# CHAINNEVERLIU/Pytorch-RL-EnhancedStableBaselines

Hardware: AMD Instinct MI355X
Metric: env-steps/sec (SAC, two-series CSTR, 4096 vec-envs) at 1/2/4/8 GPUs (higher is better)
Workload: dtype f32; 1 GPU; SAC MlpPolicy class defaults on 4096 vectorised two-series CSTR envs per GPU (obs 4/act 2, euler, batch 256, ring 244x4096, 1 gradient step per vec-step; hipGraph replay, 8 iterations per graph); n_envs_per_gpu=4096, global_batch=256, parallelism=dp1, hip_graph=True, hip_graph_requested=True, graph_unroll=8, blas=rocblas, n_updates=2370

## Files before the change

### include/cstr_rl_hip.h

```cpp
#ifndef CSTR_RL_HIP_H
#define CSTR_RL_HIP_H

#include <stdint.h>

#ifdef __cplusplus
extern "C" {
#endif

#define CSTR_ABI_VERSION 5

#define CSTR_OK 0
#define CSTR_E_BADARG (-1)
#define CSTR_E_UNSUPPORTED (-2)

#define CSTR_INTEGRATOR_EULER 0
#define CSTR_INTEGRATOR_RK4 1

typedef void *cstr_stream_t;

typedef struct cstr_coef {
    float q_v1, q_v2, cf, tf, tcf, k0, neg_e, r_gas, hk, rho_cp, cool1, cool2, neg_ua1, neg_ua2, rho_c, c_pc, dt;
    float s_lo[4], s_hi[4], s_span[4];
    float a_lo[2], a_hi[2], a_span[2];
    float target_c2, conc_span;
// ... 198 lines not shown

int cstr_sac_alpha_f32(const float *log_alpha, const float *logp, float target_entropy, float *grad_out, float *ent_coef_out,
                       float *loss_out, float *loss_sum, float *ent_coef_sum, int64_t batch, cstr_stream_t stream);

int cstr_twin_q_loss_f32(const float *q1, const float *q2, const float *target, float scale, float *gq1, float *gq2,
                         float *loss_out, float *loss_sum, int64_t batch, cstr_stream_t stream);

typedef struct cstr_alpha_part {
    const float *log_alpha;
    const float *logp_pi;
    float target_entropy;
    float *grad_out;
    float *ent_coef_out;
    float *loss_out;
    float *loss_sum;
    float *ent_coef_sum;
} cstr_alpha_part_t;
int cstr_td_twin_q_loss_f32(const float *q1_t, const float *q2_t, const float *next_logp, const float *rew, const float *done,
                            const float *ent_coef, float gamma, const float *q1, const float *q2, float scale, float *target_out,
                            float *gq1, float *gq2, float *loss_out, float *loss_sum, const cstr_alpha_part_t *alpha,
                            int64_t batch, cstr_stream_t stream);

typedef struct cstr_head_root {
    int32_t mode, batch;
    float gamma, scale;
    const float *q1_t, *q2_t, *next_logp, *rew, *done;
    const float *ent_coef;
    const float *q1, *q2;
    float *target_out;
    const float *logp;
    float *g_logp;
    float *loss_out, *loss_sum;
    cstr_alpha_part_t alpha;
} cstr_head_root_t;
int cstr_hidden_head_bwd_root_f32(const cstr_head_root_t *root, const float *y, int act, const float *w2, float *dz, float *gb1,
                                  float *gw2, float *gb2, int64_t m, int64_t k, cstr_stream_t stream);

int cstr_sac_actor_loss_f32(const float *logp, const float *q1, const float *q2, const float *ent_coef, float *g_logp, float *gq1,
                            float *gq2, float *loss_out, float *loss_sum, int64_t batch, cstr_stream_t stream);

#define CSTR_MAX_ENS_CRITICS 16
int cstr_td_ens_q_loss_f32(const float *q_t, int64_t q_t_stride, const float *next_logp, const float *rew, const float *done,
                           const float *ent_coef, float gamma, const float *q, int64_t q_stride, float scale, float *target_out, float *gq,
                           float *loss_out, float *loss_sum, const cstr_alpha_part_t *alpha, int n_critics, int64_t batch,
                           cstr_stream_t stream);
int cstr_sac_actor_ens_loss_f32(const float *logp, const float *q, int64_t q_stride, const float *ent_coef, float *g_logp, float *gq,
                                float *loss_out, float *loss_sum, int n_critics, int64_t batch, cstr_stream_t stream);

#define CSTR_SDE_MAX_LATENT 4096
#define CSTR_SDE_MAX_MATS 65537
int cstr_sde_draw_f32(const float *log_std, int log_std_cols, int latent, int act_dim, int use_expln, int64_t n_mats, float *std_out,
                      float *z, int64_t z_keep, float *mats, uint64_t *rng_ctl, cstr_stream_t stream);
int cstr_sde_head_fwd_f32(const float *h, int64_t ldh, int64_t batch, int latent, int act_dim, const float *w_mu, const float *b_mu,
                          float clip_mean, const float *mats, int64_t mat_stride, const float *std_mat, float *action, int64_t action_stride,
                          float *logp, float *aux, cstr_stream_t stream);
int cstr_sde_head_bwd_f32(const float *g_action, int64_t g_action_stride, const float *g_logp, const float *action, int64_t action_stride,
                          const float *aux, const float *h, int64_t ldh, int64_t batch, int latent, int act_dim, const float *w_mu,
                          float clip_mean, const float *mats, int64_t mat_stride, const float *std_mat, int below_act, float *g_pre,
                          float *g_x, float *g_var, float *dh, cstr_stream_t stream);
int cstr_sde_param_grad_f32(const float *h, int64_t ldh, int64_t batch, int latent, int act_dim, const float *g_pre, const float *g_x,
                            const float *g_var, const float *z, const float *std_mat, const float *log_std, int log_std_cols, int use_expln,
                            float *dw_mu, float *db_mu, float *dlog_std, cstr_stream_t stream);

int cstr_neg_mean_loss_f32(const float *q, float *gq, float *loss_out, float *loss_sum, int64_t batch, cstr_stream_t stream);

typedef struct cstr_adam_opt {
    const int64_t *adam_ctl;
    const double *lr;
    double beta1, beta2, eps;
    float grad_scale;
    int32_t reserved;
} cstr_adam_opt_t;
typedef struct cstr_wgrad_adam_set {
    cstr_wgrad_set_t g;
    float *w, *w_m, *w_v;
    float *b, *b_m, *b_v;
    float *shadow;
    int32_t opt, reserved;
    float *w_target, *b_target;
    float tau, reserved2;
} cstr_wgrad_adam_set_t;
int cstr_linear_bwd_weight_adam_sets_f32(const cstr_wgrad_adam_set_t *sets, int n_sets, const cstr_adam_opt_t *opts, int n_opts,
                                         const cstr_adam_seg_t *flat, int n_flat, cstr_stream_t stream);

#define CSTR_CHAIN_MAX_NETS 16
#define CSTR_CHAIN_MAX_WIDTH 512

typedef struct cstr_chain_net {
    const float *w1, *b1, *w2, *b2, *w3, *b3;
    const float *x;
    float *h1, *h2;
    float *q_part;
    int32_t role, reserved;
} cstr_chain_net_t;
#define CSTR_CHAIN_ROLE_PLAIN 0
#define CSTR_CHAIN_ROLE_STORE_PI 1
#define CSTR_CHAIN_ROLE_NEXT 2
#define CSTR_CHAIN_ROLE_NEXT_STORE 3
#define CSTR_CHAIN_ROLE_PI 4
#define CSTR_CHAIN_ROWS_PAIR 0
#define CSTR_CHAIN_ROWS_NEXT 1
#define CSTR_CHAIN_ROWS_OBS 2
#define CSTR_CHAIN_HEAD_GAUSSIAN 0
#define CSTR_CHAIN_HEAD_DETERMINISTIC 1

typedef struct cstr_sac_actor {
    int32_t obs_dim, act_dim, h1, h2;
    const float *w1, *b1, *w2, *b2, *hw, *hb;
} cstr_sac_actor_t;

int cstr_sac_actor_chain_fwd_f32(const cstr_sac_actor_t *actor, const cstr_ring_t *ring, int64_t *ring_ctl, int advance_ring,
                                 const int32_t *sample_idx, int64_t batch, float *x_data, float *x_pi, float *x_next, float *out_done,
                                 float *out_rew, float *a_h1, float *a_h2, float *head_part, const uint64_t *head_rng_ctl,
                                 uint64_t head_rng_offset, float *eps_all, int rows_mode, int head_n, int tiles, cstr_stream_t stream);

typedef struct cstr_sac_head_fin {
    const float *head_part;
    const float *hb;
    const float *eps;
    int32_t n_parts, act_dim, obs_dim, kind;
    int32_t part_rows, next_offset;
    float sigma, clip;
    float *x_pi, *x_next;
    float *params, *logp_pi, *logp_next;
} cstr_sac_head_fin_t;

int cstr_q_chain_fwd_f32(const cstr_chain_net_t *nets, int n_nets, int w_in, int obs_dim, int h1, int h2, int64_t batch,
                         const cstr_sac_head_fin_t *fin, int tiles, cstr_stream_t stream);

typedef struct cstr_chain_root {
    int32_t mode, batch;
    float gamma, scale;
    const float *q_part[4];
    const float *b3[4];
    int32_t n_parts, reserved;
    const float *next_logp, *rew, *done;
    const float *ent_coef;
    const float *logp;
    float *target_out;
    float *q_out;
    float *gq_out;
    float *loss_out, *loss_sum;
    cstr_alpha_part_t alpha;
    uint64_t *rng_ctl;
    uint64_t rng_advance;
    int64_t *adam_advance[2];
    double adam_beta1[2], adam_beta2[2];
} cstr_chain_root_t;
int cstr_q_chain_bwd_f32(const cstr_chain_net_t *nets, int n_nets, const cstr_chain_root_t *root, int w_in, int obs_dim, int h1, int h2,
                         float *dz2, float *dz1, float *gact_part, int tiles, cstr_stream_t stream);

int cstr_chain_sum_parts_f32(const float *part, int n_parts, int64_t rows, int cols, float *out, int64_t out_stride, cstr_stream_t stream);

int cstr_sac_actor_chain_bwd_f32(const cstr_sac_actor_t *actor, const float *gact_part, int n_nets, int n_parts, const float *ent_coef,
                                 const float *x_pi, const float *params, const float *eps, const float *a_h1, const float *a_h2,
                                 float *g_params, float *dz2, float *dz1, int64_t batch, int kind, int tiles, cstr_stream_t stream);

#define CSTR_BCQ_MAX_LATENT 256
#define CSTR_BCQ_MAX_ACT 64
#define CSTR_BCQ_MAX_SAMPLES 4096
#define CSTR_BCQ_MAX_ROWS 16777216
int cstr_bcq_latent_fwd_f32(const float *params, int64_t ldp, const float *obs, int64_t ldo, const float *eps_in, uint64_t *rng_ctl,
                            float *xdec, int64_t ldx, float *std_out, float *eps_out, int64_t batch, int obs_dim, int latent,
                            cstr_stream_t stream);
int cstr_bcq_vae_loss_f32(const float *recon, int64_t ldr, const float *act, int64_t lda, const float *params, int64_t ldp,
                          const float *std, int64_t batch, int act_dim, int latent, float *g_recon, float *g_mean, float *g_std,
// ... 92 lines not shown
```

### pytorch-rl-enhancedstablebaselines_amd/core/_native.py

```python
import ctypes as C
import os
from typing import Optional

_PKG_ROOT = os.path.dirname(os.path.dirname(os.path.abspath(__file__)))
LIB_PATH = os.environ.get("CSTR_LIB_PATH", os.path.join(_PKG_ROOT, "libcstr_rl_hip.so"))

INTEGRATORS = {"euler": 0, "rk4": 1}
RING_CTL_WORDS, ADAM_CTL_WORDS, MT_STATE_WORDS, PCG_STATE_WORDS, MAX_SAMPLE_BATCH = 4, 4, 628, 4, 16384
MAX_NOISE_PERIOD = 8
VECNORM_STATE_WORDS = 20
RNG_CTL_WORDS, MAX_HEAD_ACT, MAX_LINEAR_SETS, MAX_ADAM_SEGS = 16, 4, 16, 4
MAX_ENS_CRITICS = 16
SDE_MAX_LATENT, SDE_MAX_MATS = 4096, 65537
BCQ_MAX_LATENT, BCQ_MAX_ACT, BCQ_MAX_SAMPLES, BCQ_MAX_ROWS = 256, 64, 4096, 1 << 24
ROLLOUT_CTL_WORDS, PPO_WS_WORDS, PPO_MAX_BLOCKS, PPO_MAX_ROWS = 4, 1024, 64, 1 << 30
DQN_MAX_LEVELS = 16

SYMBOLS = (
    "cstr_abi_version", "cstr_error_string", "cstr_default_coef", "cstr_vec_step_f32", "cstr_reset_draw_f32",
    "cstr_replay_add_f32", "cstr_collect_step_f32", "cstr_collect_step_rng_f32", "cstr_mt19937_seed", "cstr_mt19937_normal_f32", "cstr_mt19937_normal_f64", "cstr_replay_sample_mt19937_f32", "cstr_replay_sample_packed_mt19937_f32", "cstr_replay_gather_packed_f32", "cstr_rollout_step_f32", "cstr_linear_act_fwd_gather_f32",
    "cstr_adam_multi_f32", "cstr_gaussian_head_fwd_f32", "cstr_gaussian_head_gemm_fwd_f32", "cstr_gaussian_head_bwd_f32", "cstr_gaussian_head_bwd_input_f32", "cstr_linear_act_fwd_f32", "cstr_linear_act_fwd_sets_f32", "cstr_linear_bwd_input_f32", "cstr_linear_bwd_weight_f32", "cstr_linear_bwd_weight_sets_f32", "cstr_td_twin_q_loss_f32", "cstr_policy_rows_fwd_f32", "cstr_policy_swizzle_f32", "cstr_target_smooth_f32", "cstr_linear_smooth_fwd_f32", "cstr_hidden_head_fwd_f32", "cstr_hidden_head_bwd_f32", "cstr_hidden_head_bwd_root_f32", "cstr_vecnorm_init_f64", "cstr_vecnorm_step_f64", "cstr_vecnorm_apply_f32",
    "cstr_td_target_min_f32", "cstr_polyak_f32", "cstr_adam_f32", "cstr_bias_act_fwd_f32", "cstr_bias_act_bwd_f32", "cstr_bias_act_bwd_rows_f32",
    "cstr_squashed_gaussian_fwd_f32", "cstr_squashed_gaussian_bwd_f32", "cstr_sac_alpha_f32", "cstr_twin_q_loss_f32",
    "cstr_sac_actor_loss_f32", "cstr_neg_mean_loss_f32", "cstr_td_ens_q_loss_f32", "cstr_sac_actor_ens_loss_f32",
    "cstr_sac_actor_chain_fwd_f32", "cstr_q_chain_fwd_f32", "cstr_q_chain_bwd_f32", "cstr_sac_actor_chain_bwd_f32",
    "cstr_linear_bwd_weight_adam_sets_f32", "cstr_chain_sum_parts_f32",
    "cstr_sde_draw_f32", "cstr_sde_head_fwd_f32", "cstr_sde_head_bwd_f32", "cstr_sde_param_grad_f32",
    "cstr_bcq_latent_fwd_f32", "cstr_bcq_vae_loss_f32", "cstr_bcq_latent_bwd_f32", "cstr_bcq_expand_f32", "cstr_bcq_perturb_fwd_f32",
    "cstr_bcq_perturb_bwd_f32", "cstr_bcq_target_f32", "cstr_bcq_select_f32",
    "cstr_diag_gaussian_act_f32", "cstr_rollout_add_f32", "cstr_gae_f32", "cstr_ppo_gather_f32", "cstr_ppo_loss_f32", "cstr_grad_clip_f32",
    "cstr_a2c_loss_f32", "cstr_rmsprop_f32",
    "cstr_mt19937_rand_flag_f64", "cstr_dqn_act_f32", "cstr_dqn_loss_f32",
    "cstr_eval_episodes_f32",
)


class Coef(C.Structure):
    _fields_ = [(n, C.c_float) for n in (
        "q_v1", "q_v2", "cf", "tf", "tcf", "k0", "neg_e", "r_gas", "hk", "rho_cp", "cool1", "cool2", "neg_ua1",
        "neg_ua2", "rho_c", "c_pc", "dt")] + [
        ("s_lo", C.c_float * 4), ("s_hi", C.c_float * 4), ("s_span", C.c_float * 4),
        ("a_lo", C.c_float * 2), ("a_hi", C.c_float * 2), ("a_span", C.c_float * 2),
        ("target_c2", C.c_float), ("conc_span", C.c_float), ("max_steps", C.c_int32)]


class Ring(C.Structure):
    _fields_ = [(n, C.c_void_p) for n in ("obs", "next_obs", "act", "rew", "done", "timeout")] + [
        ("rows", C.c_int64), ("n_envs", C.c_int64), ("obs_dim", C.c_int32), ("act_dim", C.c_int32)]


class AdamSeg(C.Structure):
    _fields_ = [("param", C.c_void_p), ("grad", C.c_void_p), ("exp_avg", C.c_void_p), ("exp_avg_sq", C.c_void_p),
                ("adam_ctl", C.c_void_p), ("lr", C.c_void_p), ("beta1", C.c_double), ("beta2", C.c_double), ("eps", C.c_double),
                ("grad_scale", C.c_float), ("n", C.c_int64), ("polyak_source", C.c_void_p), ("tau", C.c_double),
                ("shadow", C.c_void_p), ("shadow_begin", C.c_int64), ("shadow_n", C.c_int64), ("shadow_k", C.c_int64), ("own_target", C.c_void_p)]


class LinearSet(C.Structure):
    _fields_ = [("x", C.c_void_p), ("ldx", C.c_int64), ("w", C.c_void_p), ("bias", C.c_void_p), ("y", C.c_void_p), ("ldy", C.c_int64)]


class WgradSet(C.Structure):
    _fields_ = [("dz", C.c_void_p), ("x", C.c_void_p), ("ldx", C.c_int64), ("dw", C.c_void_p), ("db", C.c_void_p),
                ("m", C.c_int64), ("n", C.c_int64), ("k", C.c_int64)]


class AlphaPart(C.Structure):
    _fields_ = [("log_alpha", C.c_void_p), ("logp_pi", C.c_void_p), ("target_entropy", C.c_float), ("grad_out", C.c_void_p),
                ("ent_coef_out", C.c_void_p), ("loss_out", C.c_void_p), ("loss_sum", C.c_void_p), ("ent_coef_sum", C.c_void_p)]


class HeadRoot(C.Structure):
    _fields_ = [("mode", C.c_int32), ("batch", C.c_int32), ("gamma", C.c_float), ("scale", C.c_float), ("q1_t", C.c_void_p),
                ("q2_t", C.c_void_p), ("next_logp", C.c_void_p), ("rew", C.c_void_p), ("done", C.c_void_p), ("ent_coef", C.c_void_p),
                ("q1", C.c_void_p), ("q2", C.c_void_p), ("target_out", C.c_void_p), ("logp", C.c_void_p), ("g_logp", C.c_void_p),
                ("loss_out", C.c_void_p), ("loss_sum", C.c_void_p), ("alpha", AlphaPart)]


class PolicyMlp(C.Structure):
    _fields_ = [("k0", C.c_int32), ("h1", C.c_int32), ("h2", C.c_int32), ("act_dim", C.c_int32), ("act", C.c_int32), ("head", C.c_int32),
                ("out_act", C.c_int32), ("reserved", C.c_int32), ("w1", C.c_void_p), ("b1", C.c_void_p), ("w2", C.c_void_p),
                ("b2", C.c_void_p), ("w3", C.c_void_p), ("b3", C.c_void_p), ("w2_swizzled", C.c_void_p)]


CHAIN_MAX_NETS, CHAIN_MAX_WIDTH = 16, 512
CHAIN_ROLE_PLAIN, CHAIN_ROLE_STORE_PI, CHAIN_ROLE_NEXT, CHAIN_ROLE_NEXT_STORE, CHAIN_ROLE_PI = 0, 1, 2, 3, 4
CHAIN_ROWS_PAIR, CHAIN_ROWS_NEXT, CHAIN_ROWS_OBS = 0, 1, 2
CHAIN_HEAD_GAUSSIAN, CHAIN_HEAD_DETERMINISTIC = 0, 1


class ChainNet(C.Structure):
    _fields_ = [(n, C.c_void_p) for n in ("w1", "b1", "w2", "b2", "w3", "b3", "x", "h1", "h2", "q_part")] + [("role", C.c_int32), ("reserved", C.c_int32)]


class SacActorNet(C.Structure):
    _fields_ = [(n, C.c_int32) for n in ("obs_dim", "act_dim", "h1", "h2")] + [(n, C.c_void_p) for n in ("w1", "b1", "w2", "b2", "hw", "hb")]


class SacHeadFin(C.Structure):
    _fields_ = [(n, C.c_void_p) for n in ("head_part", "hb", "eps")] + [(n, C.c_int32) for n in ("n_parts", "act_dim", "obs_dim", "kind", "part_rows",
                                                                                                 "next_offset")] + [
        ("sigma", C.c_float), ("clip", C.c_float)] + [(n, C.c_void_p) for n in ("x_pi", "x_next", "params", "logp_pi", "logp_next")]


class ChainRoot(C.Structure):
    _fields_ = [("mode", C.c_int32), ("batch", C.c_int32), ("gamma", C.c_float), ("scale", C.c_float), ("q_part", C.c_void_p * 4),
                ("b3", C.c_void_p * 4), ("n_parts", C.c_int32), ("reserved", C.c_int32)] + [
        (n, C.c_void_p) for n in ("next_logp", "rew", "done", "ent_coef", "logp", "target_out", "q_out", "gq_out", "loss_out", "loss_sum")] + [
        ("alpha", AlphaPart), ("rng_ctl", C.c_void_p), ("rng_advance", C.c_uint64), ("adam_advance", C.c_void_p * 2),
# ... 91 lines not shown
```

### pytorch-rl-enhancedstablebaselines_amd/csrc/cstr_adam_device.h

```cpp
#pragma once
#include <hip/hip_runtime.h>
#include <stdint.h>

#include "cstr_device.h"

namespace {

__device__ __forceinline__ float polyak1(float p, float t, float tau, float om) { return __fmaf_rn(tau, p, t * om); }


struct AdamScalars { float step_size_neg, bc2_sqrt, w1, b2, omb2, eps, gscale; };

__device__ __forceinline__ void adam1(float &p, float g, float &m, float &v, const AdamScalars &a)
{
    g = g * a.gscale;
    m = __fmaf_rn(a.w1, g - m, m);
    v = __fmaf_rn(a.omb2 * g, g, v * a.b2);
    const float denom = sqrtf(v) / a.bc2_sqrt + a.eps;
    p = p + (a.step_size_neg * m) / denom;
}

struct AdamShadow { float4 *out; int64_t begin4, end4; int k, kc; };

__device__ __forceinline__ void adam_body(float *__restrict__ param, const float *__restrict__ grad, float *__restrict__ exp_avg,
// ... 30 lines not shown
    const AdamScalars a = sa;
    typedef float v4f __attribute__((ext_vector_type(4)));
    auto update = [&](const int64_t i, float4 p, float4 m, float4 v, const float4 g, float4 t) {
        adam1(p.x, g.x, m.x, v.x, a); adam1(p.y, g.y, m.y, v.y, a);
        adam1(p.z, g.z, m.z, v.z, a); adam1(p.w, g.w, m.w, v.w, a);
        p4[i] = p; m4[i] = m; v4[i] = v;
        if (own_target) {
            t.x = polyak1(p.x, t.x, tau, om); t.y = polyak1(p.y, t.y, tau, om);
            t.z = polyak1(p.z, t.z, tau, om); t.w = polyak1(p.w, t.w, tau, om);
            reinterpret_cast<float4 *>(own_target)[i] = t;
        }
        if (sh.out && i >= sh.begin4 && i < sh.end4) {
            const int64_t e = (i - sh.begin4) * 4;
            const int row = (int)(e / sh.k), col = (int)(e - (int64_t)row * sh.k);
            sh.out[((int64_t)(row >> 4) * sh.kc + (col >> 4)) * 64 + (row & 15) + 16 * ((col & 15) >> 2)] = p;
        }
    };
    if (stream_out) {
        int64_t i = tid;
        for (; i + stride < nv; i += 2 * stride) {
            const int64_t j = i + stride;
            v4f p0 = __builtin_nontemporal_load(reinterpret_cast<const v4f *>(p4 + i)), p1 = __builtin_nontemporal_load(reinterpret_cast<const v4f *>(p4 + j));
            v4f m0 = __builtin_nontemporal_load(reinterpret_cast<const v4f *>(m4 + i)), m1 = __builtin_nontemporal_load(reinterpret_cast<const v4f *>(m4 + j));
            v4f v0 = __builtin_nontemporal_load(reinterpret_cast<const v4f *>(v4 + i)), v1 = __builtin_nontemporal_load(reinterpret_cast<const v4f *>(v4 + j));
            const v4f g0 = __builtin_nontemporal_load(reinterpret_cast<const v4f *>(g4 + i)), g1 = __builtin_nontemporal_load(reinterpret_cast<const v4f *>(g4 + j));
#pragma unroll
            for (int e = 0; e < 4; ++e) {
                float pp = p0[e], mm = m0[e], vv = v0[e];
                adam1(pp, g0[e], mm, vv, a);
                p0[e] = pp; m0[e] = mm; v0[e] = vv;
                pp = p1[e]; mm = m1[e]; vv = v1[e];
                adam1(pp, g1[e], mm, vv, a);
                p1[e] = pp; m1[e] = mm; v1[e] = vv;
            }
            __builtin_nontemporal_store(p0, reinterpret_cast<v4f *>(p4 + i)); __builtin_nontemporal_store(p1, reinterpret_cast<v4f *>(p4 + j));
            __builtin_nontemporal_store(m0, reinterpret_cast<v4f *>(m4 + i)); __builtin_nontemporal_store(m1, reinterpret_cast<v4f *>(m4 + j));
            __builtin_nontemporal_store(v0, reinterpret_cast<v4f *>(v4 + i)); __builtin_nontemporal_store(v1, reinterpret_cast<v4f *>(v4 + j));
        }
        for (; i < nv; i += stride) {
            float4 p = p4[i], m = m4[i], v = v4[i];
            const float4 g = g4[i];
            adam1(p.x, g.x, m.x, v.x, a); adam1(p.y, g.y, m.y, v.y, a);
            adam1(p.z, g.z, m.z, v.z, a); adam1(p.w, g.w, m.w, v.w, a);
            p4[i] = p; m4[i] = m; v4[i] = v;
        }
    } else {
        if (first) update(tid, fp, fm, fv, fg, ft);
        for (int64_t i = tid + stride; i < nv; i += stride)
            update(i, p4[i], m4[i], v4[i], g4[i], own_target ? reinterpret_cast<const float4 *>(own_target)[i] : fp);
    }
    for (int64_t i = (nv << 2) + tid; i < n; i += stride) {
        float p = param[i], m = exp_avg[i], v = exp_avg_sq[i];
        adam1(p, grad[i], m, v, a);
        param[i] = p; exp_avg[i] = m; exp_avg_sq[i] = v;
        if (own_target) own_target[i] = polyak1(p, own_target[i], tau, om);
    }
    if (pre_advanced) return;
    if (last_block_ticket(reinterpret_cast<unsigned long long *>(adam_ctl + 1)) && threadIdx.x == 0) {
        double *pw = reinterpret_cast<double *>(adam_ctl + 2);
        adam_ctl[0] += 1;
        pw[0] *= beta1;
        pw[1] *= beta2;
    }
}


__device__ __forceinline__ void polyak_body(const float *__restrict__ param, float *__restrict__ target, const float tau,
                                            const float om, const int64_t n, const int64_t bid = blockIdx.x, const int64_t nblk = gridDim.x)
{
    const int64_t nv = n >> 2;
    const float4 *p4 = reinterpret_cast<const float4 *>(param);
    float4 *t4 = reinterpret_cast<float4 *>(target);
    const int64_t tid = bid * (int64_t)blockDim.x + threadIdx.x, stride = nblk * (int64_t)blockDim.x;
    for (int64_t i = tid; i < nv; i += stride) {
        const float4 p = p4[i];
        float4 t = t4[i];
        t.x = polyak1(p.x, t.x, tau, om); t.y = polyak1(p.y, t.y, tau, om);
        t.z = polyak1(p.z, t.z, tau, om); t.w = polyak1(p.w, t.w, tau, om);
        t4[i] = t;
    }
    for (int64_t i = (nv << 2) + tid; i < n; i += stride) target[i] = polyak1(param[i], target[i], tau, om);
}

__device__ __forceinline__ AdamScalars adam_scalars_advanced(const int64_t *adam_ctl, const double *lr, const double beta1, const double beta2,
                                                             const double eps, const float gscale)
{
    const double *pw = reinterpret_cast<const double *>(adam_ctl + 2);
    const double bc1 = 1.0 - pw[0], bc2 = 1.0 - pw[1];
    AdamScalars a;
    a.step_size_neg = -(float)(lr[0] / bc1);
    a.bc2_sqrt = (float)sqrt(bc2);
    a.w1 = (float)(1.0 - beta1);
    a.b2 = (float)beta2;
    a.omb2 = (float)(1.0 - beta2);
    a.eps = (float)eps;
    a.gscale = gscale;
    return a;
}

}
```

### pytorch-rl-enhancedstablebaselines_amd/csrc/cstr_mlp.hip

```cpp
#include <hip/hip_runtime.h>
#include <stdint.h>
#include <stdlib.h>
#include <type_traits>

#include "../../include/cstr_rl_hip.h"
#include "cstr_device.h"
#include "cstr_env_device.h"
#include "cstr_mt_device.h"
#include "cstr_rng_device.h"
#include "cstr_adam_device.h"
#include "cstr_policy_device.h"

namespace {

#ifndef CSTR_BWD_FLY
#define CSTR_BWD_FLY 4
#endif


template <int ACT>
__global__ void bias_act_fwd_kernel(float *__restrict__ y, const float *__restrict__ bias, const int64_t total, const int n,
                                    const int64_t gsz)
{
    for (int64_t i = blockIdx.x * (int64_t)blockDim.x + threadIdx.x; i < total; i += (int64_t)gridDim.x * blockDim.x) {
// ... 510 lines not shown
#pragma unroll
        for (int e = 0; e < 4; ++e)
            if (n0 + 4 * h + e < N) out[(int64_t)e * K] = acc[e];
        if (ADAM) {
            const AdamScalars a = adam_sc;
            WA_STAMP(4);
#pragma unroll
            for (int e = 0; e < 4; ++e) {
                const int row = n0 + 4 * h + e, colk = k0 + r;
                if (row < N) {
                    const int64_t i = (int64_t)row * K + colk;
                    adam1(pw[e], acc[e], pm[e], pv[e], a);
                    ad->w[i] = pw[e]; ad->w_m[i] = pm[e]; ad->w_v[i] = pv[e];
                    if (ad->w_target) ad->w_target[i] = polyak1(pw[e], pt[e], ad->tau, 1.0f - ad->tau);
                    if (ad->shadow)
                        ad->shadow[(((int64_t)(row >> 4) * ((K + 15) >> 4) + (colk >> 4)) * 64 + (row & 15) + 16 * ((colk & 15) >> 2)) * 4 + (colk & 3)] = pw[e];
                }
            }
        }
    }
    if (want_db && lane < 16 && n_ok) {
        float sum = 0.0f;
#pragma unroll
        for (int v = 0; v < WAVES; ++v) sum += (colpart[v][lane] + colpart[v][lane + 16]) + (colpart[v][lane + 32] + colpart[v][lane + 48]);
        db[g * N + n0 + lane] = sum;
        if (ADAM) {
            adam1(bw, sum, bm, bvv, adam_sc);
            ad->b[n0 + lane] = bw; ad->b_m[n0 + lane] = bm; ad->b_v[n0 + lane] = bvv;
            if (ad->b_target) ad->b_target[n0 + lane] = polyak1(bw, bt, ad->tau, 1.0f - ad->tau);
        }
    }
    WA_STAMP(5);
}

template <int WAVES, bool BUF>
__global__ __launch_bounds__(64 * WAVES) void linear_bwd_weight_kernel(const float *__restrict__ dz, const float *__restrict__ x,
                                                                       const int64_t x_group_stride, const int ldx,
                                                                       float *__restrict__ dw, float *__restrict__ db, const int M,
                                                                       const int N, const int K)
{
    const int64_t g = blockIdx.z;
    linear_bwd_weight_tile<WAVES, BUF>(dz + g * (int64_t)M * N, x + g * x_group_stride, ldx, dw, db, M, N, K, g);
}

struct WgradSets { cstr_wgrad_set_t s[CSTR_MAX_LINEAR_SETS]; };

template <int WAVES, bool BUF>
__global__ __launch_bounds__(64 * WAVES) void linear_bwd_weight_sets_kernel(const WgradSets sets)
{
    const cstr_wgrad_set_t &q = sets.s[blockIdx.z];
    if ((int64_t)blockIdx.x * 16 >= q.k || (int64_t)blockIdx.y * 16 >= q.n) return;
    linear_bwd_weight_tile<WAVES, BUF>(q.dz, q.x, (int)q.ldx, q.dw, q.db, (int)q.m, (int)q.n, (int)q.k, 0);
}

struct WgradAdamSets {
    cstr_wgrad_adam_set_t s[CSTR_MAX_LINEAR_SETS];
    cstr_adam_opt_t o[CSTR_MAX_ADAM_SEGS];
    cstr_adam_seg_t f[CSTR_MAX_ADAM_SEGS];
    int first[CSTR_MAX_LINEAR_SETS + CSTR_MAX_ADAM_SEGS + 1];
    int n_sets, n_flat;
};

template <int WAVES, bool BUF>
__global__ __launch_bounds__(64 * WAVES) void linear_bwd_weight_adam_sets_kernel(const WgradAdamSets sets)
{
    const int b = blockIdx.x, n_slices = sets.n_sets + sets.n_flat;
    int i = 0;
    while (i + 1 < n_slices && b >= sets.first[i + 1]) ++i;
    const int local = b - sets.first[i], count = sets.first[i + 1] - sets.first[i];
    if (i >= sets.n_sets) {
        const cstr_adam_seg_t &f = sets.f[i - sets.n_sets];
        if (f.polyak_source) { polyak_body(f.polyak_source, f.param, (float)f.tau, (float)(1.0 - f.tau), f.n, local, count); return; }
        adam_body(f.param, f.grad, f.exp_avg, f.exp_avg_sq, f.adam_ctl, f.lr, f.beta1, f.beta2, f.eps, f.grad_scale, f.n, AdamShadow{nullptr, 0, 0, 4, 1},
                  f.own_target, (float)f.tau, (float)(1.0 - f.tau), true, local, count);
        return;
    }
    const cstr_wgrad_adam_set_t &q = sets.s[i];
    const int kt = (int)((q.g.k + 15) >> 4);
    const cstr_adam_opt_t &o = sets.o[q.opt];
    const AdamTile ad = {q.w, q.w_m, q.w_v, q.b, q.b_m, q.b_v, q.shadow, o.adam_ctl, o.lr, o.beta1, o.beta2, o.eps, o.grad_scale,
                         q.w_target, q.b_target, q.tau};
    linear_bwd_weight_tile<WAVES, BUF, true>(q.g.dz, q.g.x, (int)q.g.ldx, q.g.dw, q.g.db, (int)q.g.m, (int)q.g.n, (int)q.g.k, 0, &ad, local % kt,
                                             local / kt);
}

template <int ACT, bool VEC4>
__global__ __launch_bounds__(256) void hidden_head_fwd_kernel(float *__restrict__ z, const float *__restrict__ b1,
                                                              const float *__restrict__ w2, const float *__restrict__ b2,
                                                              float *__restrict__ q, const int64_t rows, const int m, const int k)
{
    const int lane = threadIdx.x & 63;
    const int64_t row = blockIdx.x * (int64_t)(blockDim.x >> 6) + (threadIdx.x >> 6);
    if (row >= rows) return;
    const int64_t g = row / m;
    float *zr = z + row * k;
    const float *br = b1 + g * k, *wr = w2 + g * k;
    float acc = 0.0f;
    if (VEC4) {
        for (int c = lane * 4; c < k; c += 256) {
            float4 v = *reinterpret_cast<const float4 *>(zr + c);
            const float4 b = *reinterpret_cast<const float4 *>(br + c), w = *reinterpret_cast<const float4 *>(wr + c);
            v.x += b.x; v.y += b.y; v.z += b.z; v.w += b.w;
            if (ACT == ACT_RELU) { v.x = fmaxf(v.x, 0.0f); v.y = fmaxf(v.y, 0.0f); v.z = fmaxf(v.z, 0.0f); v.w = fmaxf(v.w, 0.0f); }
            if (ACT == ACT_TANH) { v.x = tanhf(v.x); v.y = tanhf(v.y); v.z = tanhf(v.z); v.w = tanhf(v.w); }
            *reinterpret_cast<float4 *>(zr + c) = v;
            acc += (v.x * w.x + v.y * w.y) + (v.z * w.z + v.w * w.w);
        }
    } else {
        for (int c = lane; c < k; c += 64) {
            float v = zr[c] + br[c];
            if (ACT == ACT_RELU) v = fmaxf(v, 0.0f);
            if (ACT == ACT_TANH) v = tanhf(v);
            zr[c] = v;
            acc += v * wr[c];
        }
    }
#pragma unroll
    for (int o = 32; o > 0; o >>= 1) acc += __shfl_xor(acc, o, 64);
    if (lane == 0) q[row] = acc + b2[g];
}

template <int ACT, int WAVES>
__global__ __launch_bounds__(WAVES * 64) void hidden_head_bwd_kernel(const float *__restrict__ gq, const float *__restrict__ y,
                                                                     const float *__restrict__ w2, float *__restrict__ dz,
                                                                     float *__restrict__ gb1, float *__restrict__ gw2,
                                                                     float *__restrict__ gb2, const int m, const int k)
{
    __shared__ float part[3][WAVES][64];
    const int lane = threadIdx.x & 63, wave = threadIdx.x >> 6;
    const int col = blockIdx.x * 64 + lane;
    const int64_t g = blockIdx.y, goff = g * (int64_t)m * k;
    gq += g * m;
    y += goff;
    dz += goff;
    const float w = col < k ? w2[g * k + col] : 0.0f;
    float s_b1 = 0.0f, s_w2 = 0.0f, s_b2 = 0.0f;
    constexpr int FLY = 8;
    for (int r0 = wave; r0 < m; r0 += FLY * WAVES) {
        float t[FLY], u[FLY];
#pragma unroll
        for (int j = 0; j < FLY; ++j) {
            const int r = r0 + j * WAVES;
            t[j] = (r < m && col < k) ? y[(int64_t)r * k + col] : 0.0f;
            u[j] = r < m ? gq[r] : 0.0f;
        }
#pragma unroll
        for (int j = 0; j < FLY; ++j) {
            const int r = r0 + j * WAVES;
            float d = u[j] * w;
            if (ACT == ACT_RELU) d = t[j] > 0.0f ? d : 0.0f;
            if (ACT == ACT_TANH) d = d * (1.0f - t[j] * t[j]);
            if (r < m && col < k) dz[(int64_t)r * k + col] = d;
            s_b1 += d;
            s_w2 += u[j] * t[j];
            s_b2 += u[j];
        }
    }
    part[0][wave][lane] = s_b1;
    part[1][wave][lane] = s_w2;
    part[2][wave][lane] = s_b2;
    __syncthreads();
    if (wave == 0 && gw2) {
        float a = 0.0f, b = 0.0f, c = 0.0f;
#pragma unroll
        for (int v = 0; v < WAVES; ++v) { a += part[0][v][lane]; b += part[1][v][lane]; c += part[2][v][lane]; }
        if (col < k) {
// ... 1754 lines not shown
#undef GL
#undef GL2
    return (int)hipGetLastError();
}

extern "C" int cstr_linear_smooth_fwd_f32(const float *x, int64_t ldx, const float *w, const float *bias, int act, const float *noise,
                                          uint64_t *rng_ctl, float sigma, float clip, float *out, int64_t out_stride, int64_t m, int64_t n,
                                          int64_t k, cstr_stream_t stream)
{
    if (!x || !w || !bias || !out || m <= 0 || n <= 0 || k <= 0 || ldx < k || out_stride < n) return CSTR_E_BADARG;
    if ((noise == nullptr) == (rng_ctl == nullptr)) return CSTR_E_BADARG;
    if (!(sigma >= 0.0f) || !(clip >= 0.0f) || act < 0 || act > 2) return CSTR_E_BADARG;
    if (n > 16 || k <= 32 || k > 0x7fffff || (m + 15) / 16 > 2048 || m * ldx >= (1 << 28)) return CSTR_E_UNSUPPORTED;
    const unsigned grid = (unsigned)((m + 15) / 16);
    const bool vec = (k & 3) == 0 && (ldx & 3) == 0 && aligned16(x) && aligned16(w);
    hipStream_t s = (hipStream_t)stream;
#define LS(A, V) linear_smooth_fwd_kernel<A, V><<<grid, 256, 0, s>>>(x, (int)ldx, w, bias, (int)m, (int)n, (int)k, noise, rng_ctl, sigma, clip, out, out_stride)
#define LS_ACT(V) do { if (act == 0) LS(0, V); else if (act == 1) LS(1, V); else LS(2, V); } while (0)
    if (vec) LS_ACT(true); else LS_ACT(false);
#undef LS_ACT
#undef LS
    return (int)hipGetLastError();
}

extern "C" int cstr_linear_bwd_input_f32(const float *gz, const float *w, const float *y, int act, float *dz, int64_t groups,
                                         int sum_groups, int64_t m, int64_t n, int64_t k, cstr_stream_t stream)
{
    if (!gz || !w || !dz || groups <= 0 || m <= 0 || n <= 0 || k <= 0 || (act != 0 && !y)) return CSTR_E_BADARG;
    if (act < 0 || act > 2 || m > 0x7fffff || n > 0x7fffff || k > 0x7fffff || groups > 65535 || (m + 15) / 16 > 65535) return CSTR_E_UNSUPPORTED;
    const dim3 grid((unsigned)((k + 15) / 16), (unsigned)((m + 15) / 16), (unsigned)(sum_groups ? 1 : groups));
    const int n_sum = sum_groups ? (int)groups : 0;
    const bool vec = (n & 3) == 0 && aligned16(gz);
    const bool buf = m * n < (1 << 28) && n * k < (1 << 28) && m * k < (1 << 28);
    hipStream_t s = (hipStream_t)stream;
#define LBI(A, V, W) do { if (buf) linear_bwd_input_kernel<A, V, W, true><<<grid, 64 * W, 0, s>>>(gz, w, y, dz, (int)m, (int)n, (int)k, n_sum); \
                          else linear_bwd_input_kernel<A, V, W, false><<<grid, 64 * W, 0, s>>>(gz, w, y, dz, (int)m, (int)n, (int)k, n_sum); } while (0)
#define LBI_ACT(V, W) do { if (act == 0) LBI(0, V, W); else if (act == 1) LBI(1, V, W); else LBI(2, V, W); } while (0)
    if (n > 32) { if (vec) LBI_ACT(true, 4); else LBI_ACT(false, 4); }
    else { if (vec) LBI_ACT(true, 1); else LBI_ACT(false, 1); }
#undef LBI_ACT
#undef LBI
    return (int)hipGetLastError();
}

extern "C" int cstr_linear_bwd_weight_f32(const float *dz, const float *x, int64_t x_group_stride, int64_t ldx, float *dw, float *db,
                                          int64_t groups, int64_t m, int64_t n, int64_t k, cstr_stream_t stream)
{
    if (!dz || !x || !dw || groups <= 0 || m <= 0 || n <= 0 || k <= 0 || ldx < k || x_group_stride < 0) return CSTR_E_BADARG;
    if (m > 0x7fffff || n > 0x7fffff || k > 0x7fffff || groups > 65535 || (n + 15) / 16 > 65535) return CSTR_E_UNSUPPORTED;
    const dim3 grid((unsigned)((k + 15) / 16), (unsigned)((n + 15) / 16), (unsigned)groups);
    hipStream_t s = (hipStream_t)stream;
    const bool buf = m * n < (1 << 28) && m * ldx < (1 << 28);
#define LBW(W, B) linear_bwd_weight_kernel<W, B><<<grid, 64 * W, 0, s>>>(dz, x, x_group_stride, (int)ldx, dw, db, (int)m, (int)n, (int)k)
    if (m > 32) { if (buf) LBW(4, true); else LBW(4, false); }
    else { if (buf) LBW(1, true); else LBW(1, false); }
#undef LBW
    return (int)hipGetLastError();
}

extern "C" int cstr_linear_bwd_weight_sets_f32(const cstr_wgrad_set_t *sets, int n_sets, cstr_stream_t stream)
{
    if (!sets || n_sets <= 0) return CSTR_E_BADARG;
    if (n_sets > CSTR_MAX_LINEAR_SETS) return CSTR_E_UNSUPPORTED;
    WgradSets t;
    int64_t kt = 1, nt = 1, m_min = INT64_MAX;
    for (int i = 0; i < n_sets; ++i) {
        const cstr_wgrad_set_t &q = sets[i];
        if (!q.dz || !q.x || !q.dw || q.m <= 0 || q.n <= 0 || q.k <= 0 || q.ldx < q.k) return CSTR_E_BADARG;
        if (q.m > 0x7fffff || q.n > 0x7fffff || q.k > 0x7fffff || (q.n + 15) / 16 > 65535) return CSTR_E_UNSUPPORTED;
        kt = kt > (q.k + 15) / 16 ? kt : (q.k + 15) / 16;
        nt = nt > (q.n + 15) / 16 ? nt : (q.n + 15) / 16;
        m_min = m_min < q.m ? m_min : q.m;
        t.s[i] = q;
    }
    const dim3 grid((unsigned)kt, (unsigned)nt, (unsigned)n_sets);
    hipStream_t s = (hipStream_t)stream;
    bool buf = true;
    for (int i = 0; i < n_sets; ++i) buf = buf && sets[i].m * sets[i].n < (1 << 28) && sets[i].m * sets[i].ldx < (1 << 28);
    if (m_min > 32) { if (buf) linear_bwd_weight_sets_kernel<4, true><<<grid, 256, 0, s>>>(t); else linear_bwd_weight_sets_kernel<4, false><<<grid, 256, 0, s>>>(t); }
    else { if (buf) linear_bwd_weight_sets_kernel<1, true><<<grid, 64, 0, s>>>(t); else linear_bwd_weight_sets_kernel<1, false><<<grid, 64, 0, s>>>(t); }
    return (int)hipGetLastError();
}

extern "C" int cstr_linear_bwd_weight_adam_sets_f32(const cstr_wgrad_adam_set_t *sets, int n_sets, const cstr_adam_opt_t *opts, int n_opts,
                                                    const cstr_adam_seg_t *flat, int n_flat, cstr_stream_t stream)
{
    if (!sets || n_sets <= 0 || !opts || n_opts <= 0 || n_flat < 0 || (n_flat > 0 && !flat)) return CSTR_E_BADARG;
    if (n_sets > CSTR_MAX_LINEAR_SETS || n_opts > CSTR_MAX_ADAM_SEGS || n_flat > CSTR_MAX_ADAM_SEGS) return CSTR_E_UNSUPPORTED;
    WgradAdamSets t;
    t.n_sets = n_sets;
    t.n_flat = n_flat;
    int64_t total = 0;
    for (int i = 0; i < n_opts; ++i) {
        if (!opts[i].adam_ctl || !opts[i].lr) return CSTR_E_BADARG;
        t.o[i] = opts[i];
    }
    for (int i = 0; i < n_sets; ++i) {
        const cstr_wgrad_adam_set_t &q = sets[i];
        if (!q.g.dz || !q.g.x || !q.g.dw || q.g.m <= 32 || q.g.n <= 0 || q.g.k <= 0 || q.g.ldx < q.g.k) return CSTR_E_BADARG;
        if (!q.w || !q.w_m || !q.w_v || q.opt < 0 || q.opt >= n_opts || (q.g.db && (!q.b || !q.b_m || !q.b_v))) return CSTR_E_BADARG;
        if ((q.w_target != nullptr) != (q.b_target != nullptr && q.g.db != nullptr) && q.g.db) return CSTR_E_BADARG;
        if (q.g.m * q.g.n >= (1 << 28) || q.g.m * q.g.ldx >= (1 << 28) || (q.g.n + 15) / 16 > 65535) return CSTR_E_UNSUPPORTED;
        t.first[i] = (int)total;
        total += ((q.g.k + 15) / 16) * ((q.g.n + 15) / 16);
        t.s[i] = q;
    }
    for (int i = 0; i < n_flat; ++i) {
        const cstr_adam_seg_t &f = flat[i];
        if (!f.param || f.n <= 0) return CSTR_E_BADARG;
        if (!f.polyak_source && (!f.grad || !f.exp_avg || !f.exp_avg_sq || !f.adam_ctl || !f.lr)) return CSTR_E_BADARG;
        if (f.shadow) return CSTR_E_UNSUPPORTED;
        if (!aligned16(f.param) || (f.polyak_source && !aligned16(f.polyak_source))) return CSTR_E_BADARG;
        t.first[n_sets + i] = (int)total;
        int64_t wgs = ((f.n + 3) / 4 + 255) / 256;
        total += wgs < 1 ? 1 : (wgs > 256 ? 256 : wgs);
        t.f[i] = f;
    }
    t.first[n_sets + n_flat] = (int)total;
    if (total > 0x7fffffff) return CSTR_E_UNSUPPORTED;
    linear_bwd_weight_adam_sets_kernel<4, true><<<dim3((unsigned)total), 256, 0, (hipStream_t)stream>>>(t);
    return (int)hipGetLastError();
}

extern "C" int cstr_gaussian_head_gemm_fwd_f32(const float *hidden, int64_t ldh, const float *w, const float *bias, float *params,
                                               float *eps, uint64_t *rng_ctl, float *action, int64_t action_stride, float *logp,
                                               int64_t batch, int act_dim, int64_t k, cstr_stream_t stream)
{
    if (!hidden || !w || !bias || !params || !eps || !action || batch <= 0 || act_dim <= 0 || k <= 0 || ldh < k || action_stride < act_dim)
        return CSTR_E_BADARG;
    if (act_dim > CSTR_MAX_HEAD_ACT || (k & 3) || (ldh & 3) || !aligned16(hidden) || !aligned16(w) || k > 0x7fffff) return CSTR_E_UNSUPPORTED;
    const int rows_per_wg = batch <= 1024 ? 4 : 16;
    const int64_t g = (batch + rows_per_wg - 1) / rows_per_wg;
    if (g > 0x7fffffff) return CSTR_E_UNSUPPORTED;
    gaussian_head_gemm_fwd_kernel<<<(unsigned)g, 64 * rows_per_wg, 0, (hipStream_t)stream>>>(hidden, w, (int)ldh, (int)k, batch, act_dim, bias, rng_ctl,
                                                                                params, eps, action, action_stride, logp);
    return (int)hipGetLastError();
}

extern "C" int cstr_linear_act_fwd_sets_f32(const cstr_linear_set_t *sets, int n_sets, int act, int64_t m, int64_t n, int64_t k,
                                            cstr_stream_t stream)
{
    if (!sets || n_sets <= 0 || m <= 0 || n <= 0 || k <= 0) return CSTR_E_BADARG;
    if (n_sets > CSTR_MAX_LINEAR_SETS || act < 0 || act > 2 || m > 0x7fffff || n > 0x7fffff || k > 0x7fffff || (m + 15) / 16 > 65535)
        return CSTR_E_UNSUPPORTED;
    LinearSets t;
    bool vec = (k & 3) == 0, buf = true;
    for (int i = 0; i < n_sets; ++i) {
        const cstr_linear_set_t &q = sets[i];
        if (!q.x || !q.w || !q.bias || !q.y || q.ldx < k || q.ldy < n) return CSTR_E_BADARG;
        vec = vec && (q.ldx & 3) == 0 && aligned16(q.x) && aligned16(q.w);
        buf = buf && m * q.ldx < (1 << 28) && n * k < (1 << 28);
        t.s[i] = q;
    }
    const dim3 grid((unsigned)((n + 15) / 16), (unsigned)((m + 15) / 16), (unsigned)n_sets);
    const bool split = k > 32 && (int64_t)grid.x * grid.y * (grid.z < 4 ? grid.z : 4) <= 2048;
    hipStream_t s = (hipStream_t)stream;
#define LIN(A, V, W) do { if (buf) linear_act_fwd_sets_kernel<A, V, W, true><<<grid, 64 * W, 0, s>>>(t, (int)m, (int)n, (int)k); \
                          else linear_act_fwd_sets_kernel<A, V, W, false><<<grid, 64 * W, 0, s>>>(t, (int)m, (int)n, (int)k); } while (0)
#define LIN_ACT(V, W) do { if (act == 0) LIN(0, V, W); else if (act == 1) LIN(1, V, W); else LIN(2, V, W); } while (0)
    if (vec) { if (split) LIN_ACT(true, 4); else LIN_ACT(true, 1); }
    else { if (split) LIN_ACT(false, 4); else LIN_ACT(false, 1); }
#undef LIN_ACT
#undef LIN
    return (int)hipGetLastError();
}
```

Before: 68.50 million env-steps/s.

## Add lean specialised wgrad+Adam kernel for 256-row batches with preloaded slice bounds

```diff
diff --git a/include/cstr_rl_hip.h b/include/cstr_rl_hip.h
--- a/include/cstr_rl_hip.h
+++ b/include/cstr_rl_hip.h
@@ -304,6 +304,8 @@
 } cstr_wgrad_adam_set_t;
 int cstr_linear_bwd_weight_adam_sets_f32(const cstr_wgrad_adam_set_t *sets, int n_sets, const cstr_adam_opt_t *opts, int n_opts,
                                          const cstr_adam_seg_t *flat, int n_flat, cstr_stream_t stream);
+int cstr_wgrad_adam_lean(int on);
+int cstr_wgrad_adam_tile_body(int64_t m, int64_t n, int64_t k, int64_t tile_n, int64_t tile_k);
 
 #define CSTR_CHAIN_MAX_NETS 16
 #define CSTR_CHAIN_MAX_WIDTH 512
diff --git a/pytorch-rl-enhancedstablebaselines_amd/core/_native.py b/pytorch-rl-enhancedstablebaselines_amd/core/_native.py
--- a/pytorch-rl-enhancedstablebaselines_amd/core/_native.py
+++ b/pytorch-rl-enhancedstablebaselines_amd/core/_native.py
@@ -24,7 +24,7 @@
     "cstr_squashed_gaussian_fwd_f32", "cstr_squashed_gaussian_bwd_f32", "cstr_sac_alpha_f32", "cstr_twin_q_loss_f32",
     "cstr_sac_actor_loss_f32", "cstr_neg_mean_loss_f32", "cstr_td_ens_q_loss_f32", "cstr_sac_actor_ens_loss_f32",
     "cstr_sac_actor_chain_fwd_f32", "cstr_q_chain_fwd_f32", "cstr_q_chain_bwd_f32", "cstr_sac_actor_chain_bwd_f32",
-    "cstr_linear_bwd_weight_adam_sets_f32", "cstr_chain_sum_parts_f32",
+    "cstr_linear_bwd_weight_adam_sets_f32", "cstr_wgrad_adam_lean", "cstr_wgrad_adam_tile_body", "cstr_chain_sum_parts_f32",
     "cstr_sde_draw_f32", "cstr_sde_head_fwd_f32", "cstr_sde_head_bwd_f32", "cstr_sde_param_grad_f32",
     "cstr_bcq_latent_fwd_f32", "cstr_bcq_vae_loss_f32", "cstr_bcq_latent_bwd_f32", "cstr_bcq_expand_f32", "cstr_bcq_perturb_fwd_f32",
     "cstr_bcq_perturb_bwd_f32", "cstr_bcq_target_f32", "cstr_bcq_select_f32",
diff --git a/pytorch-rl-enhancedstablebaselines_amd/csrc/cstr_adam_device.h b/pytorch-rl-enhancedstablebaselines_amd/csrc/cstr_adam_device.h
--- a/pytorch-rl-enhancedstablebaselines_amd/csrc/cstr_adam_device.h
+++ b/pytorch-rl-enhancedstablebaselines_amd/csrc/cstr_adam_device.h
@@ -136,13 +136,12 @@
     for (int64_t i = (nv << 2) + tid; i < n; i += stride) target[i] = polyak1(param[i], target[i], tau, om);
 }
 
-__device__ __forceinline__ AdamScalars adam_scalars_advanced(const int64_t *adam_ctl, const double *lr, const double beta1, const double beta2,
-                                                             const double eps, const float gscale)
+__device__ __forceinline__ AdamScalars adam_scalars_from(const double pow1, const double pow2, const double lr, const double beta1, const double beta2,
+                                                         const double eps, const float gscale)
 {
-    const double *pw = reinterpret_cast<const double *>(adam_ctl + 2);
-    const double bc1 = 1.0 - pw[0], bc2 = 1.0 - pw[1];
+    const double bc1 = 1.0 - pow1, bc2 = 1.0 - pow2;
     AdamScalars a;
-    a.step_size_neg = -(float)(lr[0] / bc1);
+    a.step_size_neg = -(float)(lr / bc1);
     a.bc2_sqrt = (float)sqrt(bc2);
     a.w1 = (float)(1.0 - beta1);
     a.b2 = (float)beta2;
@@ -152,4 +151,11 @@
     return a;
 }
 
+__device__ __forceinline__ AdamScalars adam_scalars_advanced(const int64_t *adam_ctl, const double *lr, const double beta1, const double beta2,
+                                                             const double eps, const float gscale)
+{
+    const double *pw = reinterpret_cast<const double *>(adam_ctl + 2);
+    return adam_scalars_from(pw[0], pw[1], lr[0], beta1, beta2, eps, gscale);
 }
+
+}
diff --git a/pytorch-rl-enhancedstablebaselines_amd/csrc/cstr_mlp.hip b/pytorch-rl-enhancedstablebaselines_amd/csrc/cstr_mlp.hip
--- a/pytorch-rl-enhancedstablebaselines_amd/csrc/cstr_mlp.hip
+++ b/pytorch-rl-enhancedstablebaselines_amd/csrc/cstr_mlp.hip
@@ -616,6 +616,168 @@
                          q.w_target, q.b_target, q.tau};
     linear_bwd_weight_tile<WAVES, BUF, true>(q.g.dz, q.g.x, (int)q.g.ldx, q.g.dw, q.g.db, (int)q.g.m, (int)q.g.n, (int)q.g.k, 0, &ad, local % kt,
                                              local / kt);
+}
+
+enum { WA_FULL = 0, WA_KNARROW = 1, WA_NNARROW = 2, WA_GENERIC = 3 };
+constexpr int WA_ROWS = 256;
+constexpr int WA_BOUNDS = 30;
+
+__host__ __device__ inline bool wa_set_lean(const int64_t m, const int64_t n, const int64_t k) { return m == WA_ROWS && n * k < (1 << 28); }
+
+__host__ __device__ inline int wa_tile_body(const bool set_lean, const int n, const int k, const int tile_n, const int tile_k)
+{
+    if (!set_lean) return WA_GENERIC;
+    const bool n_full = 16 * tile_n + 16 <= n, k_full = 16 * tile_k + 16 <= k;
+    if (n_full && k_full) return WA_FULL;
+    if (k <= 16 && n_full) return WA_KNARROW;
+    if (n <= 16 && k_full) return WA_NNARROW;
+    return WA_GENERIC;
+}
+
+struct WaSet {
+    const float *dz, *x;
+    float *dw, *db, *w, *w_m, *w_v, *b, *b_m, *b_v, *shadow, *w_target, *b_target;
+    const int64_t *adam_ctl; const double *lr;
+    double beta1, beta2, eps;
+    int ldx, m, n, k, kt, lean;
+    float tau, gscale;
+};
+struct WaSets { WaSet s[CSTR_MAX_LINEAR_SETS]; cstr_adam_seg_t f[CSTR_MAX_ADAM_SEGS]; };
+
+#ifdef CSTR_POLICY_STAMPS
+#define WAL_STAMP(i) do { if (lane == 0 && blockIdx.x < 4096) policy_stamps[(blockIdx.x * 16 + wave) * 8 + (i)] = __builtin_amdgcn_s_memtime(); } while (0)
+#else
+#define WAL_STAMP(i) do { } while (0)
+#endif
+
+struct WaLds {
+    float part[4][4][64];
+    float colpart[4][64];
+    AdamScalars sc;
+};
+
+template <bool MASKED>
+__device__ __forceinline__ void wgrad_adam_lean_tile(const WaSet &q, const int tile_k, const int tile_n, WaLds &lds)
+{
+    const int lane = threadIdx.x & 63, r = lane & 15, h = lane >> 4;
+    const int wave = __builtin_amdgcn_readfirstlane(threadIdx.x >> 6);
+    const int N = q.n, K = q.k, ldx = q.ldx;
+    const int k0 = tile_k * 16, n0 = tile_n * 16;
+    const int row = n0 + 4 * h + wave, colk = k0 + r;
+    const bool ok = !MASKED || (row < N && colk < K);
+    const bool bias_lane = q.db != nullptr && tile_k == 0 && wave == 0 && lane < 16 && (!MASKED || n0 + lane < N);
+    const int i = row * K + colk;
+    WAL_STAMP(0);
+    const double *ctl = reinterpret_cast<const double *>(q.adam_ctl + 2);
+    const double pow1 = ctl[0], pow2 = ctl[1], lr = q.lr[0];
+    float pw = 0.0f, pm = 0.0f, pv = 0.0f, pt = 0.0f, bw = 0.0f, bm = 0.0f, bvv = 0.0f, bt = 0.0f;
+    if (ok) {
+        pw = q.w[i]; pm = q.w_m[i]; pv = q.w_v[i];
+        pt = (q.w_target ? q.w_target : q.w)[i];
+    }
+    if (bias_lane) {
+        bw = q.b[n0 + lane]; bm = q.b_m[n0 + lane]; bvv = q.b_v[n0 + lane];
+        bt = (q.b_target ? q.b_target : q.b)[n0 + lane];
+    }
+    WAL_STAMP(1);
+    const __amdgpu_buffer_rsrc_t rdz = operand_rsrc(q.dz, (int64_t)WA_ROWS * N), rxx = operand_rsrc(q.x, (int64_t)(WA_ROWS - 1) * ldx + K);
+    const int ar = (MASKED && n0 + r >= N) ? 0 : r, br = (MASKED && colk >= K) ? 0 : r;
+    const int va = 4 * (4 * h * N + n0 + ar), vb = 4 * (4 * h * ldx + k0 + br);
+    float4 a[4], b[4];
+#pragma unroll
+    for (int u = 0; u < 4; ++u) {
+        const int m = 16 * wave + 64 * u;
+        a[u].x = __uint_as_float(__builtin_amdgcn_raw_buffer_load_b32(rdz, va, 4 * (m * N), 0));
+        a[u].y = __uint_as_float(__builtin_amdgcn_raw_buffer_load_b32(rdz, va, 4 * ((m + 1) * N), 0));
+        a[u].z = __uint_as_float(__builtin_amdgcn_raw_buffer_load_b32(rdz, va, 4 * ((m + 2) * N), 0));
+        a[u].w = __uint_as_float(__builtin_amdgcn_raw_buffer_load_b32(rdz, va, 4 * ((m + 3) * N), 0));
+        b[u].x = __uint_as_float(__builtin_amdgcn_raw_buffer_load_b32(rxx, vb, 4 * (m * ldx), 0));
+        b[u].y = __uint_as_float(__builtin_amdgcn_raw_buffer_load_b32(rxx, vb, 4 * ((m + 1) * ldx), 0));
+        b[u].z = __uint_as_float(__builtin_amdgcn_raw_buffer_load_b32(rxx, vb, 4 * ((m + 2) * ldx), 0));
+        b[u].w = __uint_as_float(__builtin_amdgcn_raw_buffer_load_b32(rxx, vb, 4 * ((m + 3) * ldx), 0));
+    }
+    if (threadIdx.x == 192) lds.sc = adam_scalars_from(pow1, pow2, lr, q.beta1, q.beta2, q.eps, q.gscale);
+    f32x4 acc0 = {0.0f, 0.0f, 0.0f, 0.0f}, acc1 = {0.0f, 0.0f, 0.0f, 0.0f};
+    float colsum = 0.0f;
+#pragma unroll
+    for (int u = 0; u < 4; ++u) {
+        acc0 = __builtin_amdgcn_mfma_f32_16x16x4f32(a[u].x, b[u].x, acc0, 0, 0, 0);
+        acc1 = __builtin_amdgcn_mfma_f32_16x16x4f32(a[u].y, b[u].y, acc1, 0, 0, 0);
+        acc0 = __builtin_amdgcn_mfma_f32_16x16x4f32(a[u].z, b[u].z, acc0, 0, 0, 0);
+        acc1 = __builtin_amdgcn_mfma_f32_16x16x4f32(a[u].w, b[u].w, acc1, 0, 0, 0);
+        colsum += (a[u].x + a[u].y) + (a[u].z + a[u].w);
+    }
+    const bool want_db = q.db != nullptr && tile_k == 0;
+    if (want_db) lds.colpart[wave][lane] = colsum;
+    const f32x4 acc = acc0 + acc1;
+#pragma unroll
+    for (int e = 0; e < 4; ++e) lds.part[wave][e][lane] = acc[e];
+    WAL_STAMP(2);
+    __syncthreads();
+    WAL_STAMP(3);
+    const float g = ((lds.part[0][wave][lane] + lds.part[1][wave][lane]) + lds.part[2][wave][lane]) + lds.part[3][wave][lane];
+    const AdamScalars s = lds.sc;
+    WAL_STAMP(4);
+    if (ok) {
+        q.dw[i] = g;
+        adam1(pw, g, pm, pv, s);
+        q.w[i] = pw; q.w_m[i] = pm; q.w_v[i] = pv;
+        if (q.w_target) q.w_target[i] = polyak1(pw, pt, q.tau, 1.0f - q.tau);
+        if (q.shadow)
+            q.shadow[((tile_n * q.kt + tile_k) * 64 + 4 * h + wave + 16 * (r >> 2)) * 4 + (r & 3)] = pw;
+    }
+    if (bias_lane) {
+        float sum = 0.0f;
+#pragma unroll
+        for (int v = 0; v < 4; ++v) sum += (lds.colpart[v][lane] + lds.colpart[v][lane + 16]) + (lds.colpart[v][lane + 32] + lds.colpart[v][lane + 48]);
+        q.db[n0 + lane] = sum;
+        adam1(bw, sum, bm, bvv, s);
+        q.b[n0 + lane] = bw; q.b_m[n0 + lane] = bm; q.b_v[n0 + lane] = bvv;
+        if (q.b_target) q.b_target[n0 + lane] = polyak1(bw, bt, q.tau, 1.0f - q.tau);
+    }
+    WAL_STAMP(5);
+}
+
+__global__ __launch_bounds__(256) void linear_bwd_weight_adam_sets_lean_kernel(const unsigned h0, const unsigned h1, const unsigned h2, const unsigned h3,
+                                                                               const unsigned h4, const unsigned h5, const unsigned h6, const unsigned h7,
+                                                                               const unsigned h8, const unsigned h9, const unsigned h10, const unsigned h11,
+                                                                               const unsigned h12, const unsigned h13, const unsigned h14, const unsigned h15,
+                                                                               const WaSets sets)
+{
+    const unsigned hw[16] = {h0, h1, h2, h3, h4, h5, h6, h7, h8, h9, h10, h11, h12, h13, h14, h15};
+    const unsigned b = blockIdx.x, n_sets = h0 & 0xffffu;
+    unsigned lo = 0, hi = 0, i = 0;
+#pragma unroll
+    for (int t = 0; t < WA_BOUNDS; ++t) {
+        hi = (hw[1 + (t >> 1)] >> (16 * (t & 1))) & 0xffffu;
+        if (b < hi) break;
+        lo = hi;
+        ++i;
+    }
+    const unsigned local = (b - lo) & 0xffffu, count = (hi - lo) & 0xffffu;
+    if (__builtin_expect(i < n_sets, 1)) {
+        const WaSet q = sets.s[i];
+        asm volatile("" ::"s"(q.dz), "s"(q.x), "s"(q.dw), "s"(q.db), "s"(q.w), "s"(q.w_m), "s"(q.w_v), "s"(q.b), "s"(q.b_m), "s"(q.b_v), "s"(q.shadow),
+                     "s"(q.w_target), "s"(q.b_target), "s"(q.adam_ctl), "s"(q.lr), "s"(q.beta1), "s"(q.beta2), "s"(q.eps), "s"(q.ldx), "s"(q.m),
+                     "s"(q.n), "s"(q.k), "s"(q.kt), "s"(q.lean), "s"(q.tau), "s"(q.gscale));
+        __shared__ WaLds lds;
+        const unsigned kt = (unsigned)q.kt & 0xffffu;
+        const int tile_n = (int)(local / kt), tile_k = (int)(local - (unsigned)tile_n * kt);
+        const int body = wa_tile_body(q.lean != 0, q.n, q.k, tile_n, tile_k);
+        if (__builtin_expect(body == WA_GENERIC, 0)) {
+            const AdamTile ad = {q.w, q.w_m, q.w_v, q.b, q.b_m, q.b_v, q.shadow, q.adam_ctl, q.lr, q.beta1, q.beta2, q.eps, q.gscale,
+                                 q.w_target, q.b_target, q.tau};
+            linear_bwd_weight_tile<4, true, true>(q.dz, q.x, q.ldx, q.dw, q.db, q.m, q.n, q.k, 0, &ad, tile_k, tile_n);
+            return;
+        }
+        if (__builtin_expect(body == WA_FULL, 1)) { wgrad_adam_lean_tile<false>(q, tile_k, tile_n, lds); return; }
+        wgrad_adam_lean_tile<true>(q, tile_k, tile_n, lds);
+        return;
+    }
+    const cstr_adam_seg_t &f = sets.f[i - n_sets];
+    if (f.polyak_source) { polyak_body(f.polyak_source, f.param, (float)f.tau, (float)(1.0 - f.tau), f.n, local, count); return; }
+    adam_body(f.param, f.grad, f.exp_avg, f.exp_avg_sq, f.adam_ctl, f.lr, f.beta1, f.beta2, f.eps, f.grad_scale, f.n, AdamShadow{nullptr, 0, 0, 4, 1},
+              f.own_target, (float)f.tau, (float)(1.0 - f.tau), true, local, count);
 }
 
 template <int ACT, bool VEC4>
@@ -2536,11 +2698,15 @@
     return (int)hipGetLastError();
 }
 
+static int wa_lean_enabled = 1;
+
 extern "C" int cstr_linear_bwd_weight_adam_sets_f32(const cstr_wgrad_adam_set_t *sets, int n_sets, const cstr_adam_opt_t *opts, int n_opts,
                                                     const cstr_adam_seg_t *flat, int n_flat, cstr_stream_t stream)
 {
     if (!sets || n_sets <= 0 || !opts || n_opts <= 0 || n_flat < 0 || (n_flat > 0 && !flat)) return CSTR_E_BADARG;
     if (n_sets > CSTR_MAX_LINEAR_SETS || n_opts > CSTR_MAX_ADAM_SEGS || n_flat > CSTR_MAX_ADAM_SEGS) return CSTR_E_UNSUPPORTED;
+    static_assert(CSTR_MAX_LINEAR_SETS + CSTR_MAX_ADAM_SEGS <= WA_BOUNDS, "the slice boundaries must fit the preloaded head");
+    static_assert(sizeof(WaSets) + 64 <= 4096, "kernarg segment");
     WgradAdamSets t;
     t.n_sets = n_sets;
     t.n_flat = n_flat;
@@ -2572,8 +2738,40 @@
     }
     t.first[n_sets + n_flat] = (int)total;
     if (total > 0x7fffffff) return CSTR_E_UNSUPPORTED;
-    linear_bwd_weight_adam_sets_kernel<4, true><<<dim3((unsigned)total), 256, 0, (hipStream_t)stream>>>(t);
-    return (int)hipGetLastError();
+    if (!wa_lean_enabled || total >= 0xffff) {
+        linear_bwd_weight_adam_sets_kernel<4, true><<<dim3((unsigned)total), 256, 0, (hipStream_t)stream>>>(t);
+        return (int)hipGetLastError();
+    }
+    WaSets l;
+    unsigned hw[16], bound[WA_BOUNDS];
+    for (int j = 0; j < WA_BOUNDS; ++j) bound[j] = j < n_sets + n_flat ? (unsigned)t.first[j + 1] : 0xffffu;
+    hw[0] = (unsigned)n_sets | (unsigned)n_flat << 16;
+    for (int j = 1; j < 16; ++j) hw[j] = bound[2 * j - 2] | bound[2 * j - 1] << 16;
+    for (int i = 0; i < n_sets; ++i) {
+        const cstr_wgrad_adam_set_t &q = sets[i];
+        const cstr_adam_opt_t &o = opts[q.opt];
+        l.s[i] = WaSet{q.g.dz, q.g.x, q.g.dw, q.g.db, q.w, q.w_m, q.w_v, q.b, q.b_m, q.b_v, q.shadow, q.w_target, q.b_target, o.adam_ctl, o.lr,
+                       o.beta1, o.beta2, o.eps, (int)q.g.ldx, (int)q.g.m, (int)q.g.n, (int)q.g.k, (int)((q.g.k + 15) / 16),
+                       wa_set_lean(q.g.m, q.g.n, q.g.k) ? 1 : 0, q.tau, o.grad_scale};
+    }
+    for (int i = 0; i < n_flat; ++i) l.f[i] = flat[i];
+    linear_bwd_weight_adam_sets_lean_kernel<<<dim3((unsigned)total), 256, 0, (hipStream_t)stream>>>(hw[0], hw[1], hw[2], hw[3], hw[4], hw[5], hw[6], hw[7], hw[8],
+                                                                                                   hw[9], hw[10], hw[11], hw[12], hw[13], hw[14], hw[15], l);
+    return (int)hipGetLastError();
+}
+
+extern "C" int cstr_wgrad_adam_lean(int on)
+{
+    const int was = wa_lean_enabled;
+    if (on >= 0) wa_lean_enabled = on != 0;
+    return was;
+}
+
+extern "C" int cstr_wgrad_adam_tile_body(int64_t m, int64_t n, int64_t k, int64_t tile_n, int64_t tile_k)
+{
+    if (m <= 0 || n <= 0 || k <= 0 || tile_n < 0 || tile_k < 0 || tile_n * 16 >= n || tile_k * 16 >= k) return CSTR_E_BADARG;
+    if (n > 0x7fffff || k > 0x7fffff) return CSTR_E_UNSUPPORTED;
+    return wa_tile_body(wa_set_lean(m, n, k), (int)n, (int)k, (int)tile_n, (int)tile_k);
 }
 
 extern "C" int cstr_gaussian_head_gemm_fwd_f32(const float *hidden, int64_t ldh, const float *w, const float *bias, float *params,
```

Result: faster. 71.56 million env-steps/s, median of 6 (+4.5%).
